# BICLab/Spike2Former

Hardware: AMD Instinct MI355X
Metric: fwd+bwd images/sec, 512x512 T=4 ADE20K-150 (higher is better)
Workload: dtype f32 (fp32-equivalent: bf16 hi+mid+lo split operands on bf16 MFMA, fp32 accumulate; spike maps stored as bf16, exact); 1 GPU; C2: 512x512 T=4 K=150 Meta-SpikeFormer [64, 128, 256, 360] + MaskFormer head, per-GPU batch 2; global_batch=2, parallelism=dp1, weights=random-init (name-seeded)

## Files before the change

include/s2f.h:

```cpp
#ifndef S2F_H
#define S2F_H

#include <stdint.h>

#ifdef __cplusplus
extern "C" {
#endif

#define S2F_OK 0
#define S2F_EINVAL (-1)
#define S2F_EALIGN (-2)
#define S2F_ELAUNCH (-3)

#define S2F_ABI_VERSION 40
#define S2F_STAT_SLOTS 256

int s2f_version(void);
const char* s2f_last_error(void);

void* s2f_event_create(void);
void s2f_event_destroy(void* event);
int s2f_time_next_call(void* start_event, void* stop_event);
int s2f_event_elapsed_us(void* start_event, void* stop_event, double* microseconds);

int64_t s2f_lif_mask_words(int64_t n);

int s2f_lif_fwd(const float* x, const float* v_in, void* y, float* v_out, uint64_t* mask, uint8_t* count_u8,
                uint64_t* stats, int64_t n, float vth, int D, int y_bf16, void* stream);

int s2f_lif_bwd(const float* gy, const float* gv_out, const uint64_t* mask, float* gx, int64_t n, float vth, int D,
                void* stream);
int s2f_lif_bwd_ports(const float* gy, const float* gy2, const float* gv_out, const uint64_t* mask, const float* skip, float* gx,
                      int64_t n, float vth, int D, void* stream);

int s2f_lif_leaky_fwd(const float* x, const float* v_in, void* y, float* v_out, uint64_t* mask, uint64_t* stats, int64_t n, float vth,
                      int D, float tau, int decay_input, int y_bf16, void* stream);
int s2f_lif_leaky_bwd(const float* gy, const float* gv_out, const uint64_t* mask, float* gx, float* gv_in, int64_t n, float vth, int D,
// ... 33 lines not shown
                   float* g_residual, float* dgamma, float* dbeta, int64_t N, int64_t C, int64_t L, int training,
                   float vth, int D, void* stream);
int s2f_bn_up_ok(int64_t N, int64_t C, int64_t H, int64_t W, int training, int D);
int s2f_bn_act_up_fwd(const float* z, const float* conv_bias, const double* sums, float* stat_out, float* running_mean,
                      float* running_var, int64_t* num_batches_tracked, const float* gamma, const float* beta,
                      const float* residual_lo, float* u_out, const float* v_in, void* y, float* v_out, uint64_t* mask,
                      uint64_t* stats, int64_t N, int64_t C, int64_t H, int64_t W, float momentum, float eps, int training,
                      float vth, int D, int y_bf16, void* stream);

int s2f_bn2_fused_ok(int64_t N, int64_t C, int64_t L);
int s2f_bn2_act_fwd(const float* z, const float* conv_bias, float* stat_out, float* running_mean, float* running_var,
                    int64_t* num_batches_tracked, const float* gamma, const float* beta, float momentum, float eps,
                    const float* gamma2, const float* beta2, float* running_mean2, float* running_var2,
                    int64_t* num_batches_tracked2, float momentum2, float eps2, const float* residual, float* u_out,
                    const float* v_in, void* y, float* v_out, uint64_t* mask, uint64_t* stats, int64_t N, int64_t C, int64_t L,
                    float vth, int D, int y_bf16, void* stream);
int s2f_bn2_act_bwd(const float* z, const float* conv_bias, const float* stat, const float* gamma, const float* gamma2, float eps2,
                    const float* g_u, const float* g_y, const float* g_v, const uint64_t* mask, float* gz, float* g_residual,
                    float* dgamma, float* dbeta, float* dgamma2, float* dbeta2, int64_t N, int64_t C, int64_t L, float vth, int D,
                    void* stream);

int s2f_im2col(const void* x, void* cols, int N, int C, int H, int W, int kh, int kw, int stride, int pad, int x_bf16, void* stream);
int s2f_col2im(const float* cols, float* gx, int N, int C, int H, int W, int kh, int kw, int stride, int pad, void* stream);

int s2f_dwconv_fwd(const void* x, const float* w, const float* border, float* y, int N, int C, int H, int W, int K,
                   int pad, int x_bf16, void* stream);
int64_t s2f_dwconv_stats_slots(int N, int H, int W);
int s2f_dwconv_fwd_stats(const void* x, const float* w, float* y, float* partials, int64_t P, int N, int C, int H, int W,
                         int x_bf16, void* stream);
int s2f_dwconv_bn_lif_fwd(const void* x, const float* w, const float* border, const float* running_mean, const float* running_var,
                          const float* gamma, const float* beta, float eps, float* u_out, void* y_bf16, uint64_t* stats, int N,
                          int C, int H, int W, int K, int pad, int x_bf16, float vth, int D, void* stream);
int s2f_dwconv_bwd_input(const float* gy, const float* w, float* gx, int N, int C, int H, int W, int K, int pad,
                         void* stream);
int s2f_dwconv_bwd_weight(const void* x, const float* border, const float* gy, float* gw, int N, int C, int H, int W,
                          int K, int pad, int accumulate, int x_bf16, void* stream);

int s2f_split_bf16x3(const float* w, uint16_t* w_split, int M, int K, int Mpad, int Kpad, void* stream);
int s2f_split_bf16x3_multi(const int64_t* jobs, int njobs, int64_t total_workgroups, void* stream);
int s2f_spike_gemm_fwd(const uint16_t* w_split, const float* X, const float* bias, float* Y, int batch, int M, int N,
                       int K, int Mpad, int Kpad, int terms, void* stream);
int s2f_spike_conv3x3_fwd(const uint16_t* w_split, const float* X, const float* bias, float* Y, int batch, int M, int C,
                          int H, int W, int Mpad, int Kpad, int terms, void* stream);
int s2f_spike_conv3x3_dw(const float* dY, const float* X, float* dW, int batch, int M, int C, int H, int W, int accumulate,
                         void* stream);
int s2f_conv3x3_general(const uint16_t* w_split, const float* X, float* Y, int batch, int M, int C, int H, int W, int Mpad,
// ... 241 lines not shown
```

spike2former_amd/_lib.py:

```python
import ctypes
import os

import torch

_HERE = os.path.dirname(os.path.abspath(__file__))
LIB_PATH = os.environ.get("S2F_LIB") or os.path.join(_HERE, "libs2f_hip.so")

_p, _i, _i64, _f = ctypes.c_void_p, ctypes.c_int, ctypes.c_int64, ctypes.c_float

SIGNATURES = {
    "s2f_version": (_i, []),
    "s2f_last_error": (ctypes.c_char_p, []),
    "s2f_event_create": (_p, []),
    "s2f_event_destroy": (None, [_p]),
    "s2f_time_next_call": (_i, [_p, _p]),
    "s2f_event_elapsed_us": (_i, [_p, _p, ctypes.POINTER(ctypes.c_double)]),
    "s2f_lif_mask_words": (_i64, [_i64]),
    "s2f_lif_fwd": (_i, [_p, _p, _p, _p, _p, _p, _p, _i64, _f, _i, _i, _p]),
    "s2f_lif_bwd": (_i, [_p, _p, _p, _p, _i64, _f, _i, _p]),
    "s2f_lif_bwd_ports": (_i, [_p] * 6 + [_i64, _f, _i, _p]),
    "s2f_lif_leaky_fwd": (_i, [_p, _p, _p, _p, _p, _p, _i64, _f, _i, _f, _i, _i, _p]),
    "s2f_lif_leaky_bwd": (_i, [_p, _p, _p, _p, _p, _i64, _f, _i, _f, _i, _p]),
    "s2f_sum2_lif_fwd": (_i, [_p] * 7 + [_i64] * 4 + [_f, _i, _i, _p]),
    "s2f_sum2_lif_bwd": (_i, [_p] * 5 + [_i64, _i, _p]),
    "s2f_sum2_lif_bwd_ex": (_i, [_p] * 6 + [_i64, _i, _p]),
    "s2f_sum2_lif_bwd_ports": (_i, [_p] * 9 + [_i64, _i, _p]),
    "s2f_mask_loss_fwd": (_i, [_p] * 4 + [_i64, _i, _i, _f, _f, _p]),
    "s2f_mask_loss_bwd": (_i, [_p] * 5 + [_i64, _i, _i, _f, _f, _p]),
    "s2f_scale_affine_fwd": (_i, [_p] * 5 + [_i, _p]),
    "s2f_scale_affine_bwd": (_i, [_p] * 8 + [_i, _p]),
    "s2f_lif_seq_fwd": (_i, [_p, _p, _p, _p, _p, _p, _i, _i64, _f, _i, _p]),
    "s2f_lif_seq_bwd": (_i, [_p, _p, _p, _p, _p, _i, _i64, _f, _i, _p]),
    "s2f_bn_single_pass": (_i, [_i64] * 3),
    "s2f_bn_mask_words": (_i64, [_i64] * 3),
    "s2f_bn2_fused_ok": (_i, [_i64] * 3),
    "s2f_bn2_act_fwd": (_i, [_p] * 8 + [_f, _f] + [_p] * 5 + [_f, _f] + [_p] * 7 + [_i64] * 3 + [_f, _i, _i, _p]),
    "s2f_bn2_act_bwd": (_i, [_p] * 5 + [_f] + [_p] * 10 + [_i64] * 3 + [_f, _i, _p]),
    "s2f_bn_stats": (_i, [_p] * 3 + [_i64] * 3 + [_p]),
    "s2f_bn_act_fwd": (_i, [_p] * 16 + [_i64] * 3 + [_f, _f, _i, _f, _i, _i, _p]),
    "s2f_bn_act_bwd": (_i, [_p] * 13 + [_i64] * 3 + [_i, _f, _i, _p]),
    "s2f_bn_up_ok": (_i, [_i64] * 4 + [_i, _i]),
    "s2f_bn_act_up_fwd": (_i, [_p] * 16 + [_i64] * 4 + [_f, _f, _i, _f, _i, _i, _p]),
    "s2f_im2col": (_i, [_p, _p] + [_i] * 9 + [_p]),
    "s2f_col2im": (_i, [_p, _p] + [_i] * 8 + [_p]),
    "s2f_dwconv_fwd": (_i, [_p] * 4 + [_i] * 7 + [_p]),
    "s2f_dwconv_stats_slots": (_i64, [_i] * 3),
    "s2f_dwconv_fwd_stats": (_i, [_p] * 4 + [_i64] + [_i] * 5 + [_p]),
    "s2f_dwconv_bn_lif_fwd": (_i, [_p] * 7 + [_f] + [_p] * 3 + [_i] * 7 + [_f, _i, _p]),
    "s2f_dwconv_bwd_input": (_i, [_p] * 3 + [_i] * 6 + [_p]),
    "s2f_dwconv_bwd_weight": (_i, [_p] * 4 + [_i] * 8 + [_p]),
    "s2f_split_bf16x3": (_i, [_p, _p, _i, _i, _i, _i, _p]),
    "s2f_split_bf16x3_multi": (_i, [_p, _i, _i64, _p]),
    "s2f_spike_gemm_fwd": (_i, [_p] * 4 + [_i] * 7 + [_p]),
    "s2f_upsample2x_fwd": (_i, [_p, _p, _i64, _i, _i, _p]),
    "s2f_upsample2x_sigmoid_fwd": (_i, [_p, _p, _i64, _i, _i, _p]),
    "s2f_upsample2x_bwd": (_i, [_p, _p, _i64, _i, _i, _p]),
    "s2f_upsample2x_bwd_add": (_i, [_p, _p, _p, _i64, _i, _i, _p]),
    "s2f_resize_fwd": (_i, [_p, _p, _i64, _i64] + [_i] * 8 + [_p]),
    "s2f_resize_bwd_add": (_i, [_p, _p, _p, _i64] + [_i] * 5 + [_p]),
    "s2f_seg_argmax": (_i, [_p, _p, _p, _i, _i64, _i, _f, _p]),
    "s2f_tta_accumulate": (_i, [_p, _p, _i, _i64] + [_i] * 9 + [_p]),
    "s2f_tta_finish": (_i, [_p, _p, _p, _i, _i64, _i, _f, _p]),
    "s2f_seg_hist": (_i, [_p, _i, _p, _i, _i64, _i64, _i, _i64, _i, _i, _i, _p, _p]),
    "s2f_seg_confusion": (_i, [_p, _i, _p, _i, _i64, _i64, _i, _i64, _i, _i, _i, _p, _p]),
    "s2f_aug_param_bytes": (_i, []),
    "s2f_aug_crop_stats": (_i, [_p, _i64, _p, _i, _i, _i, _i, _i, ctypes.c_double, _p, _p]),
    "s2f_aug_apply": (_i, [_p, _i64, _p, _p, _i, _i, _i] + [_f] * 6 + [_i, _f, _i, _i, _p, _p, _p]),
# ... 110 lines not shown
```

spike2former_amd/graph.py:

```python
import torch

from . import ops
from .neuron import reset_net


def _check_settings(captured):
    now = ops.cfg.snapshot()
    if now != captured:
        diff = {k: (captured[k], now[k]) for k in now if now[k] != captured.get(k)}
        raise RuntimeError(f"this hipGraph was captured under different op-layer settings (captured, now): {diff}; re-capture")


class GraphedStep:

    def __init__(self, model, loss_fn, example_input, grad_buffer=None, warmup=3, optimizer=None):
        self.model, self.loss_fn = model, loss_fn
        self.static_in = example_input.clone()
        self.grad_buffer = grad_buffer
        self.optimizer = optimizer
        if optimizer is not None:
            optimizer.sync_hyper()
        self.graph = torch.cuda.CUDAGraph()
        self.static_loss = None
        side = torch.cuda.Stream()
        side.wait_stream(torch.cuda.current_stream())
        with torch.cuda.stream(side):
            for _ in range(warmup):
                self._eager_step()
        if ops.GLUE_MODE:
            with torch.cuda.stream(side), ops.glue_mode():
                self._eager_step()
        torch.cuda.current_stream().wait_stream(side)
        ops.resplit_all(self.static_in.device)
        torch.cuda.synchronize()
        import torch.distributed as dist
        mode = "thread_local" if (dist.is_available() and dist.is_initialized()) else "global"
        with torch.cuda.graph(self.graph, capture_error_mode=mode), ops.glue_mode():
            self.static_loss = self._eager_step()
        torch.cuda.synchronize()
        self._converted = ops.conversion_state()
        self._settings = ops.cfg.snapshot()

    def _eager_step(self):
        reset_net(self.model)
        if self.grad_buffer is not None:
            self.grad_buffer.zero()
        else:
            for p in self.model.parameters():
                p.grad = None
        out = self.model(self.static_in)
        loss = self.loss_fn(*out)
        loss.backward()
        ops.wgrad_join()
        if self.grad_buffer is not None:
            self.grad_buffer.gather()
        if self.optimizer is not None:
            self.optimizer.step(sync_hyper=False)
        return loss.detach()

    def __call__(self, x=None):
        _check_settings(self._settings)
        if x is not None:
            self.static_in.copy_(x, non_blocking=True)
        if self.optimizer is not None:
# ... 12 lines not shown
        params = [p for p in grad_buffer.params]
        side = torch.cuda.Stream()
        side.wait_stream(torch.cuda.current_stream())
        with torch.cuda.stream(side):
            for _ in range(warmup):
                outs = self._forward()
                torch.autograd.grad(outs, params, [torch.ones_like(o) for o in outs], allow_unused=True)
        torch.cuda.current_stream().wait_stream(side)
        ops.resplit_all(self.static_in.device)
        torch.cuda.synchronize()
        import torch.distributed as dist
        mode = "thread_local" if (dist.is_available() and dist.is_initialized()) else "global"
        self.graph_a, self.graph_b = torch.cuda.CUDAGraph(), torch.cuda.CUDAGraph()
        pool = torch.cuda.graph_pool_handle()
        with torch.cuda.graph(self.graph_a, pool=pool, capture_error_mode=mode):
            self.outs = self._forward()
        self.grad_outs = [torch.zeros_like(o) for o in self.outs]
        with torch.cuda.graph(self.graph_b, pool=pool, capture_error_mode=mode):
            grads = torch.autograd.grad(self.outs, params, self.grad_outs, allow_unused=True)
            ops.wgrad_join()
            self.red.pack(grads)
        torch.cuda.synchronize()
        self._converted = ops.conversion_state()
        self._settings = ops.cfg.snapshot()

    def _forward(self):
        reset_net(self.model)
        self.red.zero()
        return tuple(self.model(self.static_in))

    def forward(self, x=None):
        _check_settings(self._settings)
        if x is not None:
            self.static_in.copy_(x, non_blocking=True)
        self.graph_a.replay()
        return [o.detach().requires_grad_(True) for o in self.outs]

    def backward(self, leaves):
        for buf, leaf in zip(self.grad_outs, leaves):
            if leaf.grad is None:
                buf.zero_()
            else:
                buf.copy_(leaf.grad)
        self.graph_b.replay()


class GraphedHungarianStep:
# ... 45 lines not shown
                ops.wgrad_join()
                del outs, total
        torch.cuda.current_stream().wait_stream(side)
        ops.wgrad_drop()
        ops.resplit_all(dev)
        torch.cuda.synchronize()
        import torch.distributed as dist
        mode = "thread_local" if (dist.is_available() and dist.is_initialized()) else "global"
        self.graph_a, self.graph_b = torch.cuda.CUDAGraph(), torch.cuda.CUDAGraph()
        pool = torch.cuda.graph_pool_handle()
        with torch.cuda.graph(self.graph_a, pool=pool, capture_error_mode=mode):
            self.outs = self._forward()
            self._costs(self.outs)
        with torch.cuda.graph(self.graph_b, pool=pool, capture_error_mode=mode):
            losses = self._losses(self.outs)
            grads = torch.autograd.grad(sum(losses.values()), params, allow_unused=True)
            ops.wgrad_join()
            self.red.pack(grads)
            if self.optimizer is not None:
                self.optimizer.step(sync_hyper=False)
            self.losses = {k: v.detach() for k, v in losses.items()}
        torch.cuda.synchronize()
        self._converted = ops.conversion_state()
        self._settings = ops.cfg.snapshot()

    def _capture_device(self, params, dev, warmup):
        self.status = torch.zeros(1, dtype=torch.int32, device=dev)
        self.sticky = torch.zeros(1, dtype=torch.int32, device=dev)
        self.host_status = torch.zeros(1, dtype=torch.int32).pin_memory()
        side = torch.cuda.Stream()
        side.wait_stream(torch.cuda.current_stream())
        with torch.cuda.stream(side):
            for _ in range(warmup):
                outs = self._forward()
                self._tables(outs)
                self._reduce_num_masks()
                total = sum(self._losses(outs).values())
                torch.autograd.grad(total, params, allow_unused=True)
                ops.wgrad_join()
                del outs, total
        torch.cuda.current_stream().wait_stream(side)
        ops.wgrad_drop()
        ops.resplit_all(dev)
        torch.cuda.synchronize()
        import torch.distributed as dist
        self.two_graphs = dist.is_available() and dist.is_initialized()
        mode = "thread_local" if self.two_graphs else "global"
# ... 8 lines not shown
            self.losses = {k: v.detach() for k, v in losses.items()}
            self.sticky.bitwise_or_(self.status)
            self.host_status.copy_(self.sticky, non_blocking=True)

        self.graph = torch.cuda.CUDAGraph()
        if self.two_graphs:
            self.graph_tail = torch.cuda.CUDAGraph()
            pool = torch.cuda.graph_pool_handle()
            with torch.cuda.graph(self.graph, pool=pool, capture_error_mode=mode):
                self.outs = self._forward()
                self._tables(self.outs)
            with torch.cuda.graph(self.graph_tail, pool=pool, capture_error_mode=mode):
                tail(self.outs)
        else:
            with torch.cuda.graph(self.graph, capture_error_mode=mode):
                self.outs = self._forward()
                self._tables(self.outs)
                tail(self.outs)
        torch.cuda.synchronize()
        self.sticky.zero_()
        torch.cuda.synchronize()
        self.host_status.zero_()
        self._converted = ops.conversion_state()
        self._settings = ops.cfg.snapshot()

    def _tables(self, outs):
        with torch.no_grad():
            cost, count = self.crit.costs_all_classes(outs[0], outs[1], self.static_seg)
            self.crit.match_tables_device(cost, count, out=(self.tgt_labels, self.row_class, self.num_masks, self.status))

    def _reduce_num_masks(self):
        import torch.distributed as dist
        if dist.is_available() and dist.is_initialized() and dist.get_world_size() > 1:
            dist.all_reduce(self.num_masks.div_(dist.get_world_size()))

    def _raise_for(self, word):
        if word:
            torch.cuda.current_stream().synchronize()
            word |= int(self.host_status[0])
            self.sticky.zero_()
            torch.cuda.current_stream().synchronize()
            self.host_status.zero_()
            self.crit.raise_for_status(word)

    def check(self):
        if self.assign == "device":
            torch.cuda.current_stream().synchronize()
# ... 63 lines not shown
        with torch.cuda.stream(side):
            for _ in range(warmup):
                loss = self._forward()
                grad_buffer.zero()
                torch.autograd.grad([loss], params, allow_unused=True)
                ops.wgrad_join()
        torch.cuda.current_stream().wait_stream(side)
        ops.wgrad_drop()
        ops.resplit_all(self.static_in.device)
        torch.cuda.synchronize()
        import torch.distributed as dist
        mode = "thread_local" if (dist.is_available() and dist.is_initialized()) else "global"
        self.graph_f, self.graph_b = torch.cuda.CUDAGraph(), torch.cuda.CUDAGraph()
        pool = torch.cuda.graph_pool_handle()
        with torch.cuda.graph(self.graph_f, pool=pool, capture_error_mode=mode):
            self.loss = self._forward()
        with torch.cuda.graph(self.graph_b, pool=pool, capture_error_mode=mode):
            self.red.zero()
            grads = torch.autograd.grad([self.loss], params, allow_unused=True)
            ops.wgrad_join()
            self.red.pack(grads)
        torch.cuda.synchronize()
        self._converted = ops.conversion_state()
        self._settings = ops.cfg.snapshot()

    def _forward(self):
        reset_net(self.model)
        return self.loss_fn(*self.model(self.static_in))

    def __call__(self, x=None):
        _check_settings(self._settings)
        if x is not None:
            self.static_in.copy_(x, non_blocking=True)
        self.graph_f.replay()
        self.red.wait()
        self.graph_b.replay()
        self.red.reduce_async(self.buckets)
        return self.loss

    def finish(self):
        self.red.wait()
```

spike2former_amd/ops/bn.py:

```python
import torch

from .config import cfg
from .core import *


class _BNAct(torch.autograd.Function):

    @staticmethod
    def forward(ctx, z, conv_bias, gamma, beta, residual, v_in, running_mean, running_var, nbt, training, momentum,
                eps, lif_on, want_pre, keep_v, D, vth, stats, bf16, partials=None, up_lo=None, up_skip=False):
        _need_cuda(z, conv_bias, gamma, beta, residual, v_in, up_lo)
        up_in = up_lo
        z = z.contiguous()
        N, C = z.shape[0], z.shape[1]
        L = z.numel() // (N * C)
        dev = z.device
        stat = torch.empty(3 * C, dtype=torch.float32, device=dev)
        s = _stream()
        ws = None
        single = bool(training) and bool(lib.s2f_bn_single_pass(N, C, L))
        if not (training and partials is not None and partials.dim() == 3 and partials.shape[0] == C and partials.shape[2] == 2
                and partials.shape[1] in _partial_slots(z) and (cfg.BN_PARTIALS_SINGLE or not single)):
            partials = None
        if partials is not None:
# ... 80 lines not shown
        check(lib.s2f_bn_act_bwd_ports(_ptr(z), _ptr(conv_bias), _ptr(stat), _ptr(gamma), _ptr(g_u), _ptr(g_y), _ptr(g_y2), _ptr(g_v),
                                       _ptr(mask), _ptr(ws), _ptr(gz), _ptr(g_res), _ptr(dgamma), _ptr(dbeta), N, C, L,
                                       int(training), vth, D, _stream()), "s2f_bn_act_bwd_ports")
        g_bias = None
        if has_bias:
            g_bias = None if training else gamma * stat[C:2 * C] * dbeta
        if ctx.needs_input_grad[5]:
            raise RuntimeError("gradient w.r.t. the incoming membrane is not supported by the fused BN+LIF op")
        if ctx.up is not None:
            g_lo = g_through
            if g_res is not None:
                h, w = ctx.up
                g_lo = torch.empty(N, C, h, w, dtype=torch.float32, device=dev)
                check(lib.s2f_upsample2x_bwd_add(_ptr(g_res), _ptr(None if g_through is None else g_through.contiguous()), _ptr(g_lo),
                                                 N * C, h, w, _stream()), "s2f_upsample2x_bwd_add")
            return (gz, g_bias, dgamma, dbeta, None) + (None,) * 15 + (g_lo, None)
        return (gz, g_bias, dgamma, dbeta, g_res) + (None,) * 17


def _partial_slots(z):
    N, C = z.shape[0], z.shape[1]
    out = (int(lib.s2f_bn_partials_count(N, z.numel() // (N * C))),)
    if z.dim() == 4:
        out += (int(lib.s2f_dwconv_stats_slots(N, z.shape[2], z.shape[3])),)
    return out


def bn_up_ok(z, lo, training, D=8):
    if not (training and z.dim() == 4 and lo.dim() == 4 and z.is_cuda and lo.is_cuda and z.dtype == lo.dtype == torch.float32
            and z.numel() and lo.shape[:2] == z.shape[:2] and (2 * lo.shape[2], 2 * lo.shape[3]) == tuple(z.shape[2:])):
        return False
    return bool(lib.s2f_bn_up_ok(z.shape[0], z.shape[1], z.shape[2], z.shape[3], 1, D))


def bn_act(z, conv_bias, gamma, beta, running_mean, running_var, nbt, training, momentum, eps, residual=None,
           lif=False, want_pre=True, v_in=None, keep_v=False, D=8, vth=1.0, stats=None, want_border=False, partials=None,
           residual_lo=None, lo_skip=False):
    if partials is None:
        from .gemm import stats_of
        partials = stats_of(z)
    bf16 = bool(lif) and spikes_bf16_ok(D) and z.numel() % 4 == 0
    up_lo, through = None, residual_lo
    if residual_lo is not None:
        assert residual is None
        if bn_up_ok(z, residual_lo, training, D):
            up_lo = residual_lo
        else:
# ... 128 lines not shown
```

spike2former_amd/ops/config.py:

```python
import os


class Config:
    FIELDS = ("KERNEL_EVENTS", "GRAD_SINKS", "WGRAD_STREAM", "BRANCH_STREAMS", "LONG_STREAMS", "LONG_WHAT", "SPIKES_BF16",
              "SPIKE_GEMM_TERMS", "SPIKE_GEMM_ENABLED", "SPIKE_GEMM_CHECK", "CONV3X3_IMPLICIT", "CONV3X3_IMPLICIT_MIN_PIXELS",
              "CONV3X3_DX_IMPLICIT", "DEFER_DW", "DW_PIPE", "BN_PARTIALS", "BN_PARTIALS_SINGLE", "DENSE_GROUPED", "RESPLIT_IN_GRAPH",
              "FANOUT_PORTS", "GLUE_MODE", "STRICT_GLUE", "STRICT", "GENERAL_RESIZE")
    RUNTIME = ("KERNEL_EVENTS", "GRAD_SINKS", "WGRAD_STREAM", "BRANCH_STREAMS", "LONG_STREAMS")

    def __setattr__(self, name, value):
        if name not in self.FIELDS:
            raise AttributeError(f"ops.cfg has no switch {name!r} (the switches are ops.cfg.FIELDS)")
        object.__setattr__(self, name, value)

    def __init__(self):
        self.KERNEL_EVENTS = None
        self.GRAD_SINKS = None
        self.WGRAD_STREAM = None
        self.DEFER_DW = True
        self.BRANCH_STREAMS = None
        self.LONG_STREAMS = None
        self.LONG_WHAT = ("lat", "mf", "kv")
        self.SPIKES_BF16 = True
        self.SPIKE_GEMM_TERMS = 3
        self.SPIKE_GEMM_ENABLED = True
        self.CONV3X3_IMPLICIT = True
        self.CONV3X3_IMPLICIT_MIN_PIXELS = int(os.environ.get("S2F_CONV3_MIN_PIXELS", 32 * 32))
        self.CONV3X3_DX_IMPLICIT = True
        self.DW_PIPE = os.environ.get("S2F_DW_PIPE", "1") != "0"
        self.SPIKE_GEMM_CHECK = False
        self.BN_PARTIALS = os.environ.get("S2F_BN_PARTIALS", "1") != "0"
        self.BN_PARTIALS_SINGLE = os.environ.get("S2F_BN_PARTIALS_SINGLE", "0") != "0"
        self.DENSE_GROUPED = os.environ.get("S2F_DENSE_GROUPED", "1") != "0"
        self.RESPLIT_IN_GRAPH = True
        self.FANOUT_PORTS = os.environ.get("S2F_FANOUT_PORTS", "1") != "0"
        self.GLUE_MODE = os.environ.get("S2F_GLUE_MODE", "0") != "0"
        self.STRICT_GLUE = os.environ.get("S2F_STRICT_GLUE", "0") != "0"
        self.STRICT = os.environ.get("S2F_STRICT", "0") != "0"
        self.GENERAL_RESIZE = True

    def snapshot(self):
        return {n: getattr(self, n) for n in self.FIELDS if n not in self.RUNTIME and n not in ("STRICT", "STRICT_GLUE")}


cfg = Config()
```

spike2former_amd/ops/conv.py:

```python
import torch

from .config import cfg
from .core import *
from .gemm import *


class _DWConv(torch.autograd.Function):

    @staticmethod
    def forward(ctx, x, tok, w, border, pad, stats=False):
        _need_cuda(w, border, spikes=x)
        x, w = x.contiguous(), w.contiguous()
        N, C, H, W = x.shape
        K = w.shape[-1]
        Ho, Wo = H + 2 * pad - K + 1, W + 2 * pad - K + 1
        y = torch.empty(N, C, Ho, Wo, dtype=torch.float32, device=x.device)
        if border is not None:
            border = border.contiguous()
        xb = int(x.dtype == torch.bfloat16)
        P = 0
        if stats and K == 3 and pad == 1 and border is None and _want_partials(True, N, C, H * W) and x.data_ptr() % 16 == 0:
            P = int(lib.s2f_dwconv_stats_slots(N, H, W))
        if P:
            part = torch.empty(C, P, 2, dtype=torch.float32, device=x.device)
# ... 69 lines not shown
    x = x.contiguous()
    cols = torch.empty(N, C * kh * kw, Ho * Wo, dtype=x.dtype, device=x.device)
    check(lib.s2f_im2col(_ptr(x), _ptr(cols), N, C, H, W, kh, kw, stride, padding, int(x.dtype == torch.bfloat16), _stream()),
          "s2f_im2col")
    return cols


def col2im(dcols, C, H, W, kh, kw, stride, padding):
    N = dcols.shape[0]
    if not dcols.is_cuda or dcols.dtype != torch.float32:
        raise RuntimeError("col2im: needs fp32 columns in device memory (there is no host path)")
    dcols = dcols.contiguous()
    gx = torch.empty(N, C, H, W, dtype=torch.float32, device=dcols.device)
    check(lib.s2f_col2im(_ptr(dcols), _ptr(gx), N, C, H, W, kh, kw, stride, padding, _stream()), "s2f_col2im")
    return gx


class _ConvDense(torch.autograd.Function):

    @staticmethod
    def forward(ctx, x, tok, weight, bias, stride, padding, spike_input, stats=False):
        _need_cuda(weight, bias, spikes=x)
        ctx.has_tok = tok is not None
        part = None
        xb = x.dtype == torch.bfloat16
        N, C, H, W = x.shape
        M, _, kh, kw = weight.shape
        Ho = (H + 2 * padding - kh) // stride + 1
        Wo = (W + 2 * padding - kw) // stride + 1
        w2d = weight.view(M, -1)
        implicit = (spike_input and cfg.SPIKE_GEMM_ENABLED and cfg.CONV3X3_IMPLICIT and kh == 3 and kw == 3 and stride == 1
                    and padding == 1 and C % 32 == 0 and W % 4 == 0
                    and H * W >= cfg.CONV3X3_IMPLICIT_MIN_PIXELS)
        if implicit:
            x = x.contiguous()
            if cfg.SPIKE_GEMM_CHECK:
                assert _is_spike_grid(x), "not a spike tensor"
            y = torch.empty(N, M, H * W, dtype=torch.float32, device=x.device)
            _time_next("spike_gemm_fwd", 4 * N * H * W * (C + M), 2 * N * M * H * W * C * 9,
                       moved=N * H * W * ((2 if xb else 4) * C + 4 * M))
            pg = xb and cfg.SPIKE_GEMM_TERMS == 3
            P = _want_partials(stats and pg and bias is None, N, M, H * W)
            if P:
                part = torch.empty(M, P, 2, dtype=torch.float32, device=x.device)
                check(lib.s2f_pgemm_conv3x3_bf16_stats(_ptr(pack_weight_conv3(weight)), _ptr(x), _ptr(y), _ptr(part), N, M, C, H, W,
                                                       _stream()), "s2f_pgemm_conv3x3_bf16_stats")
            elif pg:
                check(lib.s2f_pgemm_conv3x3_bf16(_ptr(pack_weight_conv3(weight)), _ptr(x), _ptr(bias), _ptr(y), N, M, C, H, W, 0,
                                                 _stream()), "s2f_pgemm_conv3x3_bf16")
            else:
                ws = split_weight_conv3(weight)
                fn = lib.s2f_spike_conv3x3_fwd_bf16 if xb else lib.s2f_spike_conv3x3_fwd
                check(fn(_ptr(ws), _ptr(x), _ptr(bias), _ptr(y), N, M, C, H, W, ws.shape[1], ws.shape[2], cfg.SPIKE_GEMM_TERMS,
                         _stream()), "s2f_spike_conv3x3_fwd")
            ctx.save_for_backward(x, weight)
            ctx.geo = (N, C, H, W, M, kh, kw, Ho, Wo, stride, padding, bias is not None, True)
            ctx.implicit = True
            part = y.new_empty(0) if part is None else part
            ctx.mark_non_differentiable(part)
            ctx.set_materialize_grads(False)
            return y.view(N, M, Ho, Wo), part
        ctx.implicit = False
        cols = im2col(x, kh, kw, stride, padding)
        use_mfma = spike_input and cfg.SPIKE_GEMM_ENABLED and cols.shape[2] % 4 == 0
        L = Ho * Wo
        if use_mfma:
            y = torch.empty(N, M, L, dtype=torch.float32, device=x.device)
            _time_next("spike_gemm_fwd", 4 * N * L * (cols.shape[1] + M), 2 * N * M * L * cols.shape[1],
                       moved=N * L * ((2 if xb else 4) * cols.shape[1] + 4 * M))
            pg = xb and L >= 8 and cfg.SPIKE_GEMM_TERMS == 3
            P = _want_partials(stats and pg and bias is None, N, M, L)
            if P:
                part = torch.empty(M, P, 2, dtype=torch.float32, device=x.device)
                check(lib.s2f_pgemm_nn_bf16_stats(_ptr(pack_weight(w2d)), _ptr(cols), _ptr(y), _ptr(part), N, M, L, cols.shape[1],
                                                  _stream()), "s2f_pgemm_nn_bf16_stats")
            elif pg:
                check(lib.s2f_pgemm_nn_bf16(_ptr(pack_weight(w2d)), _ptr(cols), _ptr(bias), _ptr(y), N, M, L, cols.shape[1],
                                            cfg.SPIKE_GEMM_TERMS, 0, _stream()), "s2f_pgemm_nn_bf16")
            else:
                ws = split_weight(w2d)
                fn = lib.s2f_spike_gemm_fwd_bf16 if xb else lib.s2f_spike_gemm_fwd
                check(fn(_ptr(ws), _ptr(cols), _ptr(bias), _ptr(y), N, M, L, cols.shape[1], ws.shape[1], ws.shape[2],
                         cfg.SPIKE_GEMM_TERMS, _stream()), "s2f_spike_gemm_fwd")
        else:
            if xb:
# ... 9 lines not shown
                else:
                    check(lib.s2f_pgemm_dx_f32(_ptr(pack_weight(w2d, transposed=True)), _ptr(cols), 0, _ptr(y), 0, N, cols.shape[1], M,
                                               L, 0.0, 0, _stream()), "s2f_pgemm_dx_f32")
            else:
                y = bmm_small(w2d.unsqueeze(0).expand(N, -1, -1), cols)
            if bias is not None:
                y = y + bias.view(1, -1, 1)
        ctx.save_for_backward(cols, weight)
        ctx.geo = (N, C, H, W, M, kh, kw, Ho, Wo, stride, padding, bias is not None, use_mfma)
        part = y.new_empty(0) if part is None else part
        ctx.mark_non_differentiable(part)
        ctx.set_materialize_grads(False)
        return y.view(N, M, Ho, Wo), part

    @staticmethod
    def backward(ctx, gy, _gpart=None):
        cols, weight = ctx.saved_tensors
        if gy is None:
            return (None,) * 8
        N, C, H, W, M, kh, kw, Ho, Wo, stride, padding, has_bias, use_mfma = ctx.geo
        gy = gy.contiguous().view(N, M, Ho * Wo)
        w2d = weight.view(M, -1)
        gx = gw = gb = None
        xb = cols.dtype == torch.bfloat16
        if ctx.needs_input_grad[0] or ctx.needs_input_grad[1]:
            if (cfg.CONV3X3_DX_IMPLICIT and kh == 3 and kw == 3 and stride == 1 and padding == 1 and M % 32 == 0 and W % 4 == 0
                    and gy.is_cuda):
                gx = torch.empty(N, C, H, W, dtype=torch.float32, device=gy.device)
                _time_next("dx_gemm", 4 * N * H * W * (C + M), 2 * N * M * H * W * C * 9)
                if C <= 64 or M >= 256:
                    check(lib.s2f_pgemm_conv3x3_f32(_ptr(pack_weight_conv3(weight, transposed=True)), _ptr(gy), _ptr(gx), N, C, M, H,
                                                    W, 0, _stream()), "s2f_pgemm_conv3x3_f32")
                else:
                    wt = split_weight_tconv3(weight)
                    check(lib.s2f_conv3x3_general(_ptr(wt), _ptr(gy), _ptr(gx), N, C, M, H, W, wt.shape[1], wt.shape[2], _stream()),
                          "s2f_conv3x3_general")
            elif M < C and stride == 1 and kh == kw and Ho == H and Wo == W:
                wt = weight.flip(2, 3).permute(1, 0, 2, 3).reshape(C, M * kh * kw)
                gcols = im2col(gy.view(N, M, Ho, Wo), kh, kw, 1, kh - 1 - padding)
                gx = bmm_small(wt.unsqueeze(0).expand(N, -1, -1), gcols).view(N, C, H, W)
            else:
                dcols = dx_gemm(w2d, gy)
                gx = col2im(dcols, C, H, W, kh, kw, stride, padding)
        if ctx.needs_input_grad[2]:
            K = w2d.shape[1]
            if ctx.implicit:
# ... 59 lines not shown
```

Baseline: 56.77 images/s.

## Add implicit 7x7 stride-2 stem conv kernels for forward and weight grad

Adds dedicated HIP kernels for the first 7x7 stride-2 conv on fp32 image input. The forward kernel stages an input patch in LDS, splits it into bf16 hi/mid/lo terms and runs MFMA with fused BN partial stats. The weight-gradient kernel accumulates per-block partials that a second kernel reduces. This skips the im2col expansion and the generic GEMM path for the stem, at the cost of a specialised path with large LDS use, limited to C<=4 and M in {8,16,32} and used only when no input gradient is needed.

```diff
diff --git a/include/s2f.h b/include/s2f.h
--- a/include/s2f.h
+++ b/include/s2f.h
@@ -12,7 +12,7 @@
 #define S2F_EALIGN (-2)
 #define S2F_ELAUNCH (-3)
 
-#define S2F_ABI_VERSION 40
+#define S2F_ABI_VERSION 41
 #define S2F_STAT_SLOTS 256
 
 int s2f_version(void);
@@ -92,6 +92,13 @@
 
 int s2f_im2col(const void* x, void* cols, int N, int C, int H, int W, int kh, int kw, int stride, int pad, int x_bf16, void* stream);
 int s2f_col2im(const float* cols, float* gx, int N, int C, int H, int W, int kh, int kw, int stride, int pad, void* stream);
+
+int64_t s2f_stem_conv7_stats_slots(int N, int H, int W);
+int64_t s2f_stem_conv7_dw_blocks(int N, int H, int W);
+int s2f_stem_conv7_fwd(const float* x, const void* wsplit, float* y, float* partials, int64_t P, int N, int C, int H, int W, int M,
+                       int Mpad, int Kpad, void* stream);
+int s2f_stem_conv7_dw(const float* x, const float* dy, float* blocks, float* dw, int N, int C, int H, int W, int M, int accumulate,
+                      void* stream);
 
 int s2f_dwconv_fwd(const void* x, const float* w, const float* border, float* y, int N, int C, int H, int W, int K,
                    int pad, int x_bf16, void* stream);
diff --git a/spike2former_amd/_lib.py b/spike2former_amd/_lib.py
--- a/spike2former_amd/_lib.py
+++ b/spike2former_amd/_lib.py
@@ -43,6 +43,10 @@
     "s2f_bn_act_up_fwd": (_i, [_p] * 16 + [_i64] * 4 + [_f, _f, _i, _f, _i, _i, _p]),
     "s2f_im2col": (_i, [_p, _p] + [_i] * 9 + [_p]),
     "s2f_col2im": (_i, [_p, _p] + [_i] * 8 + [_p]),
+    "s2f_stem_conv7_stats_slots": (_i64, [_i] * 3),
+    "s2f_stem_conv7_dw_blocks": (_i64, [_i] * 3),
+    "s2f_stem_conv7_fwd": (_i, [_p] * 4 + [_i64] + [_i] * 7 + [_p]),
+    "s2f_stem_conv7_dw": (_i, [_p] * 4 + [_i] * 6 + [_p]),
     "s2f_dwconv_fwd": (_i, [_p] * 4 + [_i] * 7 + [_p]),
     "s2f_dwconv_stats_slots": (_i64, [_i] * 3),
     "s2f_dwconv_fwd_stats": (_i, [_p] * 4 + [_i64] + [_i] * 5 + [_p]),
diff --git a/spike2former_amd/csrc/stemconv.hip b/spike2former_amd/csrc/stemconv.hip
--- /dev/null
+++ b/spike2former_amd/csrc/stemconv.hip
@@ -0,0 +1,387 @@
+#include "gemm_common.h"
+
+#pragma clang fp contract(fast)
+
+namespace {
+
+constexpr int TH = 8, TW = 64;
+constexpr int PH = 2 * TH + 5;
+constexpr int PPAIR = 68;
+constexpr int PITCH = 192;
+constexpr int THREADS = 512;
+constexpr int MAX_FWD_GROUPS = 1024;
+constexpr int MAX_DW_GROUPS = 256;
+
+struct Geo {
+  int N, C, H, W, M, Ho, Wo, tiles_x, tiles_y, tiles, per_group;
+};
+
+__device__ __forceinline__ float half_sum(float v) {
+  return v + __shfl_xor(v, 32);
+}
+
+__device__ __forceinline__ void stage_patch(const float* __restrict__ x, unsigned int* __restrict__ ps32, const Geo& g, int n, int ty,
+                                            int tx) {
+  const int iy0 = 2 * ty * TH - 3, ix0 = 2 * tx * TW - 3;
+  const int total = g.C * PH * PPAIR, tstride = g.C * PH * (PITCH / 2);
+  const float* xn = x + (int64_t)n * g.C * g.H * g.W;
+  for (int i0 = threadIdx.x; i0 < total; i0 += 4 * THREADS) {
+    float v[4][2];
+    int dst[4];
+#pragma unroll
+    for (int u = 0; u < 4; ++u) {
+      const int i = i0 + u * THREADS;
+      const int cr = i / PPAIR, p = i - cr * PPAIR;
+      const int c = cr / PH, r = cr - c * PH;
+      const int iy = iy0 + r, ix = ix0 + 2 * p;
+      const bool row_ok = i < total && iy >= 0 && iy < g.H;
+      const float* src = xn + ((int64_t)c * g.H + iy) * g.W + ix;
+      v[u][0] = (row_ok && ix >= 0 && ix < g.W) ? src[0] : 0.0f;
+      v[u][1] = (row_ok && ix + 1 >= 0 && ix + 1 < g.W) ? src[1] : 0.0f;
+      dst[u] = i < total ? cr * (PITCH / 2) + p : -1;
+    }
+#pragma unroll
+    for (int u = 0; u < 4; ++u) {
+      if (dst[u] < 0) continue;
+      unsigned int h, m, l;
+      s2f_split3x2(v[u][0], v[u][1], h, m, l);
+      ps32[dst[u]] = h;
+      ps32[tstride + dst[u]] = m;
+      ps32[2 * tstride + dst[u]] = l;
+    }
+  }
+}
+
+__global__ __launch_bounds__(THREADS) void stem_fwd_kernel(const float* __restrict__ x, const unsigned short* __restrict__ wsplit,
+                                                           float* __restrict__ y, float* __restrict__ part, Geo g, int Mpad, int Kpad,
+                                                           int P, int vec4) {
+  extern __shared__ __attribute__((aligned(16))) unsigned char smem[];
+  const int G = 7 * g.C, KS = (G + 1) / 2, AP = 16 * KS + 8;
+  unsigned short* As = reinterpret_cast<unsigned short*>(smem);
+  unsigned int* ps32 = reinterpret_cast<unsigned int*>(smem + (size_t)3 * 32 * AP * 2);
+  const int tstride = g.C * PH * (PITCH / 2);
+  float* red = reinterpret_cast<float*>(ps32 + 3 * tstride);
+  const int lane = threadIdx.x & 63, wave = threadIdx.x >> 6, l31 = lane & 31, half = lane >> 5;
+
+  for (int i = threadIdx.x; i < 3 * 32 * 16 * KS; i += THREADS) {
+    const int kk = i % (16 * KS), tm = i / (16 * KS), m = tm & 31, t = tm >> 5;
+    const int grp = kk >> 3, kx = kk & 7;
+    unsigned short v = 0;
+    if (m < g.M && grp < G && kx < 7) v = wsplit[((int64_t)t * Mpad + m) * Kpad + grp * 7 + kx];
+    As[(t * 32 + m) * AP + kk] = v;
+  }
+
+  float run_s = 0.0f, run_q = 0.0f;
+  const int first = blockIdx.x * g.per_group, last = min(first + g.per_group, g.tiles);
+  for (int tile = first; tile < last; ++tile) {
+    const int n = tile / (g.tiles_x * g.tiles_y), rem = tile - n * (g.tiles_x * g.tiles_y);
+    const int ty = rem / g.tiles_x, tx = rem - ty * g.tiles_x;
+    stage_patch(x, ps32, g, n, ty, tx);
+    __syncthreads();
+
+    f32x16 acc[2];
+#pragma unroll
+    for (int j = 0; j < 2; ++j)
+#pragma unroll
+      for (int r = 0; r < 16; ++r) acc[j][r] = 0.0f;
+    int c = 0, ky = half;
+    for (int ks = 0; ks < KS; ++ks) {
+      const bool live = 2 * ks + half < G;
+      bf16x8 wf[3], pf[3][2];
+#pragma unroll
+      for (int t = 0; t < 3; ++t) wf[t] = *reinterpret_cast<const bf16x8*>(&As[(t * 32 + l31) * AP + ks * 16 + 8 * half]);
+      const int row = live ? (c * PH + 2 * wave + ky) * (PITCH / 2) : 0;
+#pragma unroll
+      for (int t = 0; t < 3; ++t)
+#pragma unroll
+        for (int j = 0; j < 2; ++j) {
+          const unsigned int* p = ps32 + t * tstride + row + j * 32 + l31;
+          u32x4 q = {p[0], p[1], p[2], p[3]};
+          if (!live) q = u32x4{0u, 0u, 0u, 0u};
+          pf[t][j] = *reinterpret_cast<bf16x8*>(&q);
+        }
+#pragma unroll
+      for (int t = 0; t < 3; ++t)
+#pragma unroll
+        for (int tb = 0; tb < 3; ++tb)
+          if (t + tb < 3)
+#pragma unroll
+            for (int j = 0; j < 2; ++j) acc[j] = __builtin_amdgcn_mfma_f32_32x32x16_bf16(pf[tb][j], wf[t], acc[j], 0, 0, 0);
+      ky += 2;
+      if (ky >= 7) {
+        ky -= 7;
+        ++c;
+      }
+    }
+
+    const int oy = ty * TH + wave, ch = l31;
+    float s = 0.0f, q = 0.0f;
+    if (oy < g.Ho && ch < g.M) {
+      float* yrow = y + (((int64_t)n * g.M + ch) * g.Ho + oy) * g.Wo;
+#pragma unroll
+      for (int j = 0; j < 2; ++j)
+#pragma unroll
+        for (int rq = 0; rq < 4; ++rq) {
+          const int ox = tx * TW + j * 32 + 8 * rq + 4 * half;
+          if (vec4) {
+            if (ox < g.Wo) {
+              const f32x4 v = {acc[j][4 * rq], acc[j][4 * rq + 1], acc[j][4 * rq + 2], acc[j][4 * rq + 3]};
+              *reinterpret_cast<f32x4*>(yrow + ox) = v;
+#pragma unroll
+              for (int e = 0; e < 4; ++e) {
+                s += v[e];
+                q += v[e] * v[e];
+              }
+            }
+          } else {
+#pragma unroll
+            for (int e = 0; e < 4; ++e)
+              if (ox + e < g.Wo) {
+                const float v = acc[j][4 * rq + e];
+                yrow[ox + e] = v;
+                s += v;
+                q += v * v;
+              }
+          }
+        }
+    }
+    if (part) {
+      s = half_sum(s);
+      q = half_sum(q);
+      if (half == 0) {
+        red[(wave * 32 + l31) * 2] = s;
+        red[(wave * 32 + l31) * 2 + 1] = q;
+      }
+    }
+    __syncthreads();
+    if (part && threadIdx.x < 32) {
+#pragma unroll
+      for (int w = 0; w < THREADS / 64; ++w) {
+        run_s += red[(w * 32 + threadIdx.x) * 2];
+        run_q += red[(w * 32 + threadIdx.x) * 2 + 1];
+      }
+    }
+  }
+  if (part && threadIdx.x < g.M && threadIdx.x < 32) {
+    part[((int64_t)threadIdx.x * P + blockIdx.x) * 2] = run_s;
+    part[((int64_t)threadIdx.x * P + blockIdx.x) * 2 + 1] = run_q;
+  }
+}
+
+__global__ __launch_bounds__(THREADS) void stem_dw_kernel(const float* __restrict__ x, const float* __restrict__ dy,
+                                                          float* __restrict__ blocks, Geo g, int vec4) {
+  extern __shared__ __attribute__((aligned(16))) unsigned char smem[];
+  unsigned int* ps32 = reinterpret_cast<unsigned int*>(smem);
+  const unsigned short* ps16 = reinterpret_cast<const unsigned short*>(smem);
+  const int tstride16 = g.C * PH * PITCH;
+  const int lane = threadIdx.x & 63, wave = threadIdx.x >> 6, l31 = lane & 31, half = lane >> 5;
+  const int K = 49 * g.C;
+  const int NT = (K + 31) / 32;
+
+  int koff[7];
+#pragma unroll
+  for (int jt = 0; jt < 7; ++jt) {
+    const int k = jt * 32 + l31;
+    const int c = k / 49, r = k - c * 49, ky = r / 7, kx = r - ky * 7;
+    koff[jt] = k < K ? (c * PH + ky) * PITCH + kx : 0;
+  }
+  f32x16 acc[7];
+#pragma unroll
+  for (int jt = 0; jt < 7; ++jt)
+#pragma unroll
+    for (int r = 0; r < 16; ++r) acc[jt][r] = 0.0f;
+
+  const int first = blockIdx.x * g.per_group, last = min(first + g.per_group, g.tiles);
+  for (int tile = first; tile < last; ++tile) {
+    const int n = tile / (g.tiles_x * g.tiles_y), rem = tile - n * (g.tiles_x * g.tiles_y);
+    const int ty = rem / g.tiles_x, tx = rem - ty * g.tiles_x;
+    const int oy = ty * TH + wave;
+    float d[4][8];
+    {
+      const bool ok = oy < g.Ho && l31 < g.M;
+      const float* drow = dy + (((int64_t)n * g.M + (ok ? l31 : 0)) * g.Ho + (ok ? oy : 0)) * g.Wo;
+#pragma unroll
+      for (int st = 0; st < 4; ++st) {
+        const int ox = tx * TW + st * 16 + 8 * half;
+        if (vec4) {
+#pragma unroll
+          for (int h4 = 0; h4 < 2; ++h4) {
+            f32x4 v = {0.0f, 0.0f, 0.0f, 0.0f};
+            if (ok && ox + 4 * h4 < g.Wo) v = *reinterpret_cast<const f32x4*>(drow + ox + 4 * h4);
+#pragma unroll
+            for (int e = 0; e < 4; ++e) d[st][4 * h4 + e] = v[e];
+          }
+        } else {
+#pragma unroll
+          for (int e = 0; e < 8; ++e) d[st][e] = (ok && ox + e < g.Wo) ? drow[ox + e] : 0.0f;
+        }
+      }
+    }
+    __syncthreads();
+    stage_patch(x, ps32, g, n, ty, tx);
+    __syncthreads();
+
+#pragma unroll
+    for (int st = 0; st < 4; ++st) {
+      bf16x8 df[3];
+      {
+        u32x4 h, m, l;
+#pragma unroll
+        for (int e = 0; e < 4; ++e) {
+          unsigned int a, b, cc;
+          s2f_split3x2(d[st][2 * e], d[st][2 * e + 1], a, b, cc);
+          h[e] = a;
+          m[e] = b;
+          l[e] = cc;
+        }
+        df[0] = *reinterpret_cast<bf16x8*>(&h);
+        df[1] = *reinterpret_cast<bf16x8*>(&m);
+        df[2] = *reinterpret_cast<bf16x8*>(&l);
+      }
+      const int base = 2 * wave * PITCH + 2 * (st * 16 + 8 * half);
+#pragma unroll
+      for (int jt = 0; jt < 7; ++jt) {
+        if (jt >= NT) break;
+        bf16x8 pf[3];
+#pragma unroll
+        for (int t = 0; t < 3; ++t) {
+          const unsigned short* p = ps16 + t * tstride16 + koff[jt] + base;
+          u32x4 qv;
+#pragma unroll
+          for (int e = 0; e < 4; ++e) qv[e] = (unsigned int)p[4 * e] | ((unsigned int)p[4 * e + 2] << 16);
+          pf[t] = *reinterpret_cast<bf16x8*>(&qv);
+        }
+#pragma unroll
+        for (int t = 0; t < 3; ++t)
+#pragma unroll
+          for (int tb = 0; tb < 3; ++tb)
+            if (t + tb < 3) acc[jt] = __builtin_amdgcn_mfma_f32_32x32x16_bf16(df[t], pf[tb], acc[jt], 0, 0, 0);
+      }
+    }
+  }
+
+  float* buf = reinterpret_cast<float*>(smem);
+  for (int w = 1; w < THREADS / 64; ++w) {
+    __syncthreads();
+    if (wave == w) {
+#pragma unroll
+      for (int jt = 0; jt < 7; ++jt)
+        if (jt < NT)
+#pragma unroll
+          for (int r = 0; r < 16; ++r) buf[(jt * 16 + r) * 64 + lane] = acc[jt][r];
+    }
+    __syncthreads();
+    if (wave == 0) {
+#pragma unroll
+      for (int jt = 0; jt < 7; ++jt)
+        if (jt < NT)
+#pragma unroll
+          for (int r = 0; r < 16; ++r) acc[jt][r] += buf[(jt * 16 + r) * 64 + lane];
+    }
+  }
+  if (wave == 0) {
+    float* out = blocks + (int64_t)blockIdx.x * g.M * K;
+#pragma unroll
+    for (int jt = 0; jt < 7; ++jt)
+      if (jt < NT)
+#pragma unroll
+        for (int r = 0; r < 16; ++r) {
+          const int m = (r & 3) + 8 * (r >> 2) + 4 * half, k = jt * 32 + l31;
+          if (m < g.M && k < K) out[m * K + k] = acc[jt][r];
+        }
+  }
+}
+
+__global__ __launch_bounds__(256) void stem_dw_reduce_kernel(const float* __restrict__ blocks, float* __restrict__ dw, int nblocks,
+                                                             int MK, int accumulate) {
+  const int i = blockIdx.x * 256 + threadIdx.x;
+  if (i >= MK) return;
+  float s = 0.0f;
+  for (int b = 0; b < nblocks; ++b) s += blocks[(int64_t)b * MK + i];
+  dw[i] = accumulate ? dw[i] + s : s;
+}
+
+int geometry(const char* who, int N, int C, int H, int W, int M, int max_groups, Geo& g) {
+  S2F_REQUIRE(N >= 1 && H >= 1 && W >= 1, S2F_EINVAL, "%s: bad shape", who);
+  S2F_REQUIRE(C >= 1 && C <= 4, S2F_EINVAL, "%s: needs 1 <= C <= 4 input channels (got %d)", who, C);
+  S2F_REQUIRE(M == 8 || M == 16 || M == 32, S2F_EINVAL, "%s: M = %d not in {8, 16, 32}", who, M);
+  g.N = N, g.C = C, g.H = H, g.W = W, g.M = M;
+  g.Ho = (H - 1) / 2 + 1;
+  g.Wo = (W - 1) / 2 + 1;
+  g.tiles_x = (g.Wo + TW - 1) / TW;
+  g.tiles_y = (g.Ho + TH - 1) / TH;
+  const int64_t tiles = (int64_t)N * g.tiles_x * g.tiles_y;
+  S2F_REQUIRE(tiles < (1ll << 30) && (int64_t)N * (C > M ? C : M) * H * W < (1ll << 40), S2F_EINVAL, "%s: map too large", who);
+  g.tiles = (int)tiles;
+  g.per_group = (g.tiles + max_groups - 1) / max_groups;
+  return S2F_OK;
+}
+inline int groups_of(const Geo& g) { return (g.tiles + g.per_group - 1) / g.per_group; }
+
+inline size_t patch_bytes(int C) { return (size_t)3 * C * PH * PITCH * 2; }
+
+template <typename KernelT>
+int raise_lds(const char* who, KernelT kernel, bool& raised) {
+  if (raised) return S2F_OK;
+  hipError_t e = hipFuncSetAttribute(reinterpret_cast<const void*>(kernel), hipFuncAttributeMaxDynamicSharedMemorySize, 160 * 1024);
+  S2F_REQUIRE(e == hipSuccess, S2F_ELAUNCH, "%s: cannot raise the dynamic LDS limit: %s", who, hipGetErrorString(e));
+  raised = true;
+  return S2F_OK;
+}
+
+}
+
+extern "C" int64_t s2f_stem_conv7_stats_slots(int N, int H, int W) {
+  Geo g;
+  if (N < 1 || H < 1 || W < 1 || geometry("s2f_stem_conv7_stats_slots", N, 1, H, W, 8, MAX_FWD_GROUPS, g)) return 0;
+  return groups_of(g);
+}
+
+extern "C" int64_t s2f_stem_conv7_dw_blocks(int N, int H, int W) {
+  Geo g;
+  if (N < 1 || H < 1 || W < 1 || geometry("s2f_stem_conv7_dw_blocks", N, 1, H, W, 8, MAX_DW_GROUPS, g)) return 0;
+  return groups_of(g);
+}
+
+extern "C" int s2f_stem_conv7_fwd(const float* x, const void* wsplit, float* y, float* partials, int64_t P, int N, int C, int H, int W,
+                                  int M, int Mpad, int Kpad, void* stream) {
+  S2F_REQUIRE(x && wsplit && y, S2F_EINVAL, "s2f_stem_conv7_fwd: null pointer");
+  Geo g;
+  int rc = geometry("s2f_stem_conv7_fwd", N, C, H, W, M, MAX_FWD_GROUPS, g);
+  if (rc) return rc;
+  S2F_REQUIRE(Mpad >= M && Kpad >= 49 * C, S2F_EINVAL, "s2f_stem_conv7_fwd: the weight split [3][%d][%d] does not hold [%d][%d]", Mpad,
+              Kpad, M, 49 * C);
+  S2F_REQUIRE(s2f_aligned16(y), S2F_EALIGN, "s2f_stem_conv7_fwd: y must be 16-byte aligned");
+  const int groups = groups_of(g);
+  S2F_REQUIRE(!partials || P == groups, S2F_EINVAL, "s2f_stem_conv7_fwd: P must be s2f_stem_conv7_stats_slots(N, H, W)");
+  S2F_REQUIRE(!partials || (reinterpret_cast<uintptr_t>(partials) & 7u) == 0, S2F_EALIGN,
+              "s2f_stem_conv7_fwd: partials must be 8-byte aligned");
+  const int KS = (7 * C + 1) / 2;
+  const size_t lds = (size_t)3 * 32 * (16 * KS + 8) * 2 + patch_bytes(C) + (THREADS / 64) * 32 * 2 * sizeof(float);
+  static bool raised = false;
+  rc = raise_lds("s2f_stem_conv7_fwd", stem_fwd_kernel, raised);
+  if (rc) return rc;
+  S2F_LAUNCH(true, true, stem_fwd_kernel, dim3(groups), dim3(THREADS), lds, (hipStream_t)stream, x,
+             reinterpret_cast<const unsigned short*>(wsplit), y, partials, g, Mpad, Kpad, (int)P, (int)(g.Wo % 4 == 0));
+  return s2f_check_launch("s2f_stem_conv7_fwd");
+}
+
+extern "C" int s2f_stem_conv7_dw(const float* x, const float* dy, float* blocks, float* dw, int N, int C, int H, int W, int M,
+                                 int accumulate, void* stream) {
+  S2F_REQUIRE(x && dy && blocks && dw, S2F_EINVAL, "s2f_stem_conv7_dw: null pointer");
+  Geo g;
+  int rc = geometry("s2f_stem_conv7_dw", N, C, H, W, M, MAX_DW_GROUPS, g);
+  if (rc) return rc;
+  S2F_REQUIRE(s2f_aligned16(dy), S2F_EALIGN, "s2f_stem_conv7_dw: dY must be 16-byte aligned");
+  const int groups = groups_of(g), MK = M * 49 * C;
+  size_t lds = patch_bytes(C);
+  if (lds < (size_t)32 * 224 * sizeof(float)) lds = (size_t)32 * 224 * sizeof(float);
+  static bool raised = false;
+  rc = raise_lds("s2f_stem_conv7_dw", stem_dw_kernel, raised);
+  if (rc) return rc;
+  S2F_LAUNCH(true, false, stem_dw_kernel, dim3(groups), dim3(THREADS), lds, (hipStream_t)stream, x, dy, blocks, g,
+             (int)(g.Wo % 4 == 0));
+  S2F_LAUNCH(false, true, stem_dw_reduce_kernel, dim3((MK + 255) / 256), dim3(256), 0, (hipStream_t)stream,
+             (const float*)blocks, dw, groups, MK, accumulate);
+  return s2f_check_launch("s2f_stem_conv7_dw");
+}
diff --git a/spike2former_amd/graph.py b/spike2former_amd/graph.py
--- a/spike2former_amd/graph.py
+++ b/spike2former_amd/graph.py
@@ -5,7 +5,7 @@
 
 
 def _check_settings(captured):
-    now = ops.cfg.snapshot()
+    now = ops.config.settings()
     if now != captured:
         diff = {k: (captured[k], now[k]) for k in now if now[k] != captured.get(k)}
         raise RuntimeError(f"this hipGraph was captured under different op-layer settings (captured, now): {diff}; re-capture")
@@ -39,7 +39,7 @@
             self.static_loss = self._eager_step()
         torch.cuda.synchronize()
         self._converted = ops.conversion_state()
-        self._settings = ops.cfg.snapshot()
+        self._settings = ops.config.settings()
 
     def _eager_step(self):
         reset_net(self.model)
@@ -98,7 +98,7 @@
             self.red.pack(grads)
         torch.cuda.synchronize()
         self._converted = ops.conversion_state()
-        self._settings = ops.cfg.snapshot()
+        self._settings = ops.config.settings()
 
     def _forward(self):
         reset_net(self.model)
@@ -190,7 +190,7 @@
             self.losses = {k: v.detach() for k, v in losses.items()}
         torch.cuda.synchronize()
         self._converted = ops.conversion_state()
-        self._settings = ops.cfg.snapshot()
+        self._settings = ops.config.settings()
 
     def _capture_device(self, params, dev, warmup):
         self.status = torch.zeros(1, dtype=torch.int32, device=dev)
@@ -245,7 +245,7 @@
         torch.cuda.synchronize()
         self.host_status.zero_()
         self._converted = ops.conversion_state()
-        self._settings = ops.cfg.snapshot()
+        self._settings = ops.config.settings()
 
     def _tables(self, outs):
         with torch.no_grad():
@@ -355,7 +355,7 @@
             self.red.pack(grads)
         torch.cuda.synchronize()
         self._converted = ops.conversion_state()
-        self._settings = ops.cfg.snapshot()
+        self._settings = ops.config.settings()
 
     def _forward(self):
         reset_net(self.model)
diff --git a/spike2former_amd/ops/bn.py b/spike2former_amd/ops/bn.py
--- a/spike2former_amd/ops/bn.py
+++ b/spike2former_amd/ops/bn.py
@@ -126,7 +126,8 @@
     N, C = z.shape[0], z.shape[1]
     out = (int(lib.s2f_bn_partials_count(N, z.numel() // (N * C))),)
     if z.dim() == 4:
-        out += (int(lib.s2f_dwconv_stats_slots(N, z.shape[2], z.shape[3])),)
+        out += (int(lib.s2f_dwconv_stats_slots(N, z.shape[2], z.shape[3])),
+                int(lib.s2f_stem_conv7_stats_slots(N, 2 * z.shape[2], 2 * z.shape[3])))
     return out
 
 
diff --git a/spike2former_amd/ops/config.py b/spike2former_amd/ops/config.py
--- a/spike2former_amd/ops/config.py
+++ b/spike2former_amd/ops/config.py
@@ -44,3 +44,9 @@
 
 
 cfg = Config()
+
+STEM_DIRECT = True
+
+
+def settings():
+    return dict(cfg.snapshot(), STEM_DIRECT=STEM_DIRECT)
diff --git a/spike2former_amd/ops/conv.py b/spike2former_amd/ops/conv.py
--- a/spike2former_amd/ops/conv.py
+++ b/spike2former_amd/ops/conv.py
@@ -1,5 +1,6 @@
 import torch
 
+from . import config as _config
 from .config import cfg
 from .core import *
 from .gemm import *
@@ -115,6 +116,7 @@
     def forward(ctx, x, tok, weight, bias, stride, padding, spike_input, stats=False):
         _need_cuda(weight, bias, spikes=x)
         ctx.has_tok = tok is not None
+        ctx.direct = False
         part = None
         xb = x.dtype == torch.bfloat16
         N, C, H, W = x.shape
@@ -154,6 +156,27 @@
             ctx.set_materialize_grads(False)
             return y.view(N, M, Ho, Wo), part
         ctx.implicit = False
+        ctx.direct = (_config.STEM_DIRECT and not spike_input and x.dtype == torch.float32 and kh == 7 and kw == 7 and stride == 2
+                      and padding == 3 and C <= 4 and M in (8, 16, 32) and not ctx.needs_input_grad[0])
+        if ctx.direct:
+            x = x.contiguous()
+            L = Ho * Wo
+            y = torch.empty(N, M, Ho, Wo, dtype=torch.float32, device=x.device)
+            ws = split_weight(w2d)
+            P = int(lib.s2f_stem_conv7_stats_slots(N, H, W)) if _want_partials(stats and bias is None, N, M, L) else 0
+            if P:
+                part = torch.empty(M, P, 2, dtype=torch.float32, device=x.device)
+            _time_next("dx_gemm", 4 * N * L * (w2d.shape[1] + M), 2 * N * M * L * w2d.shape[1], moved=4 * N * (C * H * W + M * L))
+            check(lib.s2f_stem_conv7_fwd(_ptr(x), _ptr(ws), _ptr(y), _ptr(part), P, N, C, H, W, M, ws.shape[1], ws.shape[2],
+                                         _stream()), "s2f_stem_conv7_fwd")
+            if bias is not None:
+                y = y + bias.view(1, -1, 1, 1)
+            ctx.save_for_backward(x, weight)
+            ctx.geo = (N, C, H, W, M, kh, kw, Ho, Wo, stride, padding, bias is not None, False)
+            part = y.new_empty(0) if part is None else part
+            ctx.mark_non_differentiable(part)
+            ctx.set_materialize_grads(False)
+            return y, part
         cols = im2col(x, kh, kw, stride, padding)
         use_mfma = spike_input and cfg.SPIKE_GEMM_ENABLED and cols.shape[2] % 4 == 0
         L = Ho * Wo
@@ -209,6 +232,19 @@
         gy = gy.contiguous().view(N, M, Ho * Wo)
         w2d = weight.view(M, -1)
         gx = gw = gb = None
+        if ctx.direct:
+            if ctx.needs_input_grad[2]:
+                x = cols
+                if gy.data_ptr() % 16:
+                    gy = gy.clone()
+                sink = _sink_for(weight)
+                gw = torch.empty_like(weight) if sink is None else None
+                blocks = torch.empty(int(lib.s2f_stem_conv7_dw_blocks(N, H, W)), M, w2d.shape[1], dtype=torch.float32, device=gy.device)
+                check(lib.s2f_stem_conv7_dw(_ptr(x), _ptr(gy), _ptr(blocks), _ptr(gw if sink is None else sink), N, C, H, W, M,
+                                            int(sink is not None), _stream()), "s2f_stem_conv7_dw")
+            if has_bias and ctx.needs_input_grad[3]:
+                gb = gy.sum((0, 2))
+            return (None, None, gw, gb, None, None, None, None)
         xb = cols.dtype == torch.bfloat16
         if ctx.needs_input_grad[0] or ctx.needs_input_grad[1]:
             if (cfg.CONV3X3_DX_IMPLICIT and kh == 3 and kw == 3 and stride == 1 and padding == 1 and M % 32 == 0 and W % 4 == 0
```

After: 57.13 images/s, median of 6. Within noise of the previous version (+0.6%).
